# catid/video_stabilizer

Measured on AMD Instinct MI355X. Metric: aligned frames/sec, higher is better.
Workload: dtype u8

## Files before the change

### include/vs_amd.h

```cpp
#ifndef VS_AMD_H
#define VS_AMD_H

#include <stddef.h>
#include <stdint.h>

#ifdef __cplusplus
extern "C" {
#endif

#define VS_OK 0
#define VS_ERR_ARG (-1)
#define VS_ERR_HIP (-2)
#define VS_ERR_UNSUPPORTED (-3)
#define VS_ERR_STATE (-4)
#define VS_ERR_NOMEM (-5)

enum { VS_MEM_HOST = 0, VS_MEM_DEVICE = 1 };
enum { VS_FMT_GRAY8 = 0, VS_FMT_BGR8 = 1, VS_FMT_BGR10 = 2, VS_FMT_BGR12 = 3, VS_FMT_BGR16_FULL = 4 };
int vs_format_bits(int format);
int vs_format_max_value(int format);
enum { VS_WARP_LANCZOS2 = 0, VS_WARP_BILINEAR = 1, VS_WARP_LANCZOS2_FAST = 2, VS_WARP_LANCZOS2_SEP = 3, VS_WARP_BILINEAR_CV = 4 };
enum { VS_BORDER_CLAMP = 0, VS_BORDER_CONSTANT = 1 };
enum {
    VS_SELECT_STL_HOST = 0,
// ... 83 lines not shown
int vs_stream_retire(void* stream);
int vs_bgr_image_warp(const void* src, int w, int h, int src_stride, int channels, int bits,
                      const vs_transform* t, int mode, int border, int max_value,
                      void* dst, int dst_stride, int mem, void* stream);
int vs_bgr_image_warp_batch(const void* src, size_t src_frame_stride, int n_frames,
                            int w, int h, int src_stride, int channels, int bits,
                            const vs_transform* t , int mode, int border, int max_value,
                            void* dst, size_t dst_frame_stride, int dst_stride, int mem, void* stream);
int vs_bgr_image_warp_roi_batch(const void* src, size_t src_frame_stride, int n_frames, int w, int h, int src_stride,
                                int channels, int bits, const vs_transform* t, int mode, int border, int max_value,
                                int roi_x, int roi_y, int roi_w, int roi_h,
                                void* dst, size_t dst_frame_stride, int dst_stride, int mem, void* stream);
int vs_bgr_image_warp_fill_batch(const void* src, size_t src_frame_stride, int n_src, int w, int h, int src_stride,
                                 int channels, int bits, int n_out, int n_cand, const int32_t* cand_frame,
                                 const vs_transform* cand_t, int border, int max_value,
                                 int roi_x, int roi_y, int roi_w, int roi_h,
                                 void* dst, size_t dst_frame_stride, int dst_stride, int mem, void* stream);
typedef struct vs_fill_blend_params { int feather; int match; } vs_fill_blend_params;
int vs_bgr_channel_sums_batch(const void* src, size_t src_frame_stride, int n, int w, int h, int src_stride, int format,
                              uint64_t* sums, int mem, void* stream);
int vs_bgr_image_warp_fill_blend_batch(const void* src, size_t src_frame_stride, int n_src, int w, int h, int src_stride,
                                       int channels, int bits, int n_out, int n_cand, const int32_t* cand_frame,
                                       const vs_transform* cand_t, const uint64_t* sums, const vs_fill_blend_params* params,
                                       int border, int max_value, int roi_x, int roi_y, int roi_w, int roi_h,
                                       void* dst, size_t dst_frame_stride, int dst_stride, int mem, void* stream);
typedef struct vs_deblur_params { float sensitivity; float max_ratio; } vs_deblur_params;
void vs_deblur_params_default(vs_deblur_params* p);
int vs_bgr_sharpness_batch(const void* src, size_t src_frame_stride, int n, int w, int h, int src_stride, int format,
                           uint64_t* sharpness, int mem, void* stream);
int vs_bgr_deblur_batch(const void* src, size_t src_frame_stride, int n_src, int w, int h, int src_stride, int format,
                        const uint64_t* sharpness, int n_out, int n_cand, const int32_t* cand_frame, const vs_transform* cand_t,
                        const vs_deblur_params* params ,
                        void* dst, size_t dst_frame_stride, int dst_stride, int mem, void* stream);
typedef struct vs_denoise_params { int strength; } vs_denoise_params;
void vs_denoise_params_default(vs_denoise_params* p);
int vs_bgr_denoise_batch(const void* src, size_t src_frame_stride, int n_src, int w, int h, int src_stride, int format,
                         int n_out, int n_cand, const int32_t* cand_frame, const vs_transform* cand_t,
                         const vs_denoise_params* params ,
                         void* dst, size_t dst_frame_stride, int dst_stride, int mem, void* stream);
typedef struct vs_deflicker_params { int step; } vs_deflicker_params;
void vs_deflicker_params_default(vs_deflicker_params* p);
int vs_bgr_exposure_stats_batch(const void* src, size_t src_frame_stride, int n_src, int w, int h, int src_stride, int format,
                                int n_out, int n_cand, const int32_t* cand_frame, const vs_transform* cand_t,
                                const vs_deflicker_params* params , uint64_t* stats, int mem, void* stream);
int vs_exposure_gains_batch(const uint64_t* stats, int n_out, int n_cand, int w, int h,
                            const vs_deflicker_params* params , uint32_t* gains, int mem, void* stream);
int vs_bgr_gain_batch(const void* src, size_t src_frame_stride, int n, int w, int h, int src_stride, int format,
                      const uint32_t* gains, void* dst, size_t dst_frame_stride, int dst_stride, int mem, void* stream);
int vs_bgr_image_warp_f32(const void* src, int w, int h, int src_stride, int channels, int bits,
                          const vs_transform* t, int mode, int border,
                          float* dst, int dst_stride, int mem, void* stream);
int vs_bgr_to_gray(const void* src, int w, int h, int src_stride, int bits, int shift_to_8,
                   uint8_t* dst, int dst_stride, int mem, void* stream);

typedef struct vs_flow_params {
    double pyr_scale;
    int    levels;
    int    winsize;
    int    iterations;
    int    poly_n;
    double poly_sigma;
    int    flags;
} vs_flow_params;
void vs_flow_params_default(vs_flow_params* p);
typedef struct vs_flow vs_flow;
vs_flow* vs_flow_create(const vs_flow_params* params , int device);
void     vs_flow_destroy(vs_flow* f);
int vs_flow_compute(vs_flow* f, const uint8_t* prev, const uint8_t* next, int w, int h, int stride, int mem, float* flow,
                    int flow_stride);
int vs_flow_jitter(vs_flow* f, const void* frames, size_t frame_stride, int n, int w, int h, int stride, int format, int mem,
                   float* pair_medians, double* median);

int vs_test_fail_alloc(int k);

int vs_debug_bounds_check(void);
int vs_debug_bounds_selftest(void);

int vs_calib_copy12(const void* src_dev, void* dst_dev, size_t bytes, void* stream);
int vs_shader_clock_probe(void* stream, double* shader_mhz);

typedef struct vs_aligner vs_aligner;
typedef struct vs_align_info {
    int32_t status;
    int32_t fail_reason;
    int32_t fail_level;
    int32_t levels;
    int32_t iterations[16];
    double  condition[16];
    double  phase_dx, phase_dy, phase_response;
    int32_t selected_x[16], selected_y[16];
    vs_transform level_transform[16];
} vs_align_info;

vs_aligner* vs_aligner_create(const vs_aligner_params* params , int device);
void vs_aligner_destroy(vs_aligner* a);
int  vs_aligner_set_select_mode(vs_aligner* a, int select_mode);
int  vs_aligner_get_select_mode(const vs_aligner* a);
enum { VS_BATCH_EXCLUSIVE = 0, VS_BATCH_SHARED = 1 };
int  vs_aligner_set_batch_mode(vs_aligner* a, int batch_mode);
int  vs_aligner_reset(vs_aligner* a);
void* vs_aligner_stream(const vs_aligner* a);
int   vs_aligner_wait_stream(vs_aligner* a, void* producer_stream);
int  vs_aligner_align_next(vs_aligner* a, const void* frame, int w, int h, int stride, int format, int mem,
                           const vs_aligner_params* params, vs_transform* out);
int  vs_aligner_align_batch(vs_aligner* a, const void* frames, size_t frame_stride, int n,
                            int w, int h, int stride, int format, int mem,
// ... 63 lines not shown
```

### video_stabilizer_amd/capi.py

```python
import ctypes as C
import os

import numpy as np

_HERE = os.path.dirname(os.path.abspath(__file__))
LIB_PATH = os.environ.get("VS_AMD_LIB", os.path.join(_HERE, "libvs_amd.so"))

MEM_HOST, MEM_DEVICE = 0, 1
FMT_GRAY8, FMT_BGR8 = 0, 1
FMT_BGR10, FMT_BGR12, FMT_BGR16_FULL = 2, 3, 4
WARP_LANCZOS2, WARP_BILINEAR, WARP_LANCZOS2_FAST, WARP_LANCZOS2_SEP, WARP_BILINEAR_CV = 0, 1, 2, 3, 4
BORDER_CLAMP, BORDER_CONSTANT = 0, 1
SELECT_STL_HOST, SELECT_DEVICE, SELECT_STABLE = 0, 1, 2
BATCH_EXCLUSIVE, BATCH_SHARED = 0, 1
ABI_VERSION = 5


class Transform(C.Structure):
    _fields_ = [("A", C.c_double), ("B", C.c_double), ("TX", C.c_double), ("TY", C.c_double)]

    def tup(self):
        return (self.A, self.B, self.TX, self.TY)

    @staticmethod
# ... 83 lines not shown
    "vs_stabilizer_stream": (_vp, [_vp]),
    "vs_stabilizer_wait_stream": (_i32, [_vp, _vp]),
    "vs_aligner_params_default": (None, [C.POINTER(AlignerParams)]),
    "vs_stabilizer_params_default": (None, [C.POINTER(StabilizerParams)]),
    "vs_transform_inverse": (Transform, [_TP]),
    "vs_transform_compose": (Transform, [_TP, _TP]),
    "vs_transform_warp": (Point, [_TP, Point]),
    "vs_transform_warp_center": (Point, [_TP, Point, _f64, _f64]),
    "vs_transform_max_corner_displacement": (_f64, [_TP, _f64, _f64]),
    "vs_tile_size": (_i32, [_i32, _i32]),
    "vs_ul_params_sparse": (None, [_TP, _i32, _i32, _vp]),
    "vs_ul_params_warp": (None, [_TP, _i32, _i32, _vp]),
    "vs_cv_inverse_matrix": (None, [_TP, _i32, _i32, _vp]),
    "vs_smoother_create": (_vp, [_i32, _i32, _f64]),
    "vs_smoother_destroy": (None, [_vp]),
    "vs_smoother_update": (_i32, [_vp, _TP, _TP]),
    "vs_tvl1_smooth": (None, [_vp, _i32, _f64, _i32, _vp]),
    "vs_calib_copy12": (_i32, [_vp, _vp, _sz, _vp]),
    "vs_pyr_down": (_i32, [_vp, _i32, _i32, _i32, _vp, _i32, _i32, _i32, _i32, _vp]),
    "vs_grad_xy": (_i32, [_vp, _i32, _i32, _i32, _vp, _vp, _i32, _vp]),
    "vs_grad_argmax": (_i32, [_vp, _vp, _i32, _i32, _i32, _vp, _vp, _i32, _vp]),
    "vs_sparse_jac": (_i32, [_vp, _vp, _i32, _i32, _vp, _vp, _i32, _i32, _vp, _vp, _i32, _vp]),
    "vs_keyframe_fused": (_i32, [_vp, _i32, _i32, _i32, _i32, _vp, _vp, _vp, _vp, _i32, _vp]),
    "vs_sparse_warpdiff": (_i32, [_vp, _vp, _i32, _i32, _i32, _vp, _i32, _i32, _f32, _f32, _f32, _f32, _vp, _i32, _vp]),
    "vs_sparse_ica": (_i32, [_vp, _vp, _i32, _i32, _i32, _vp, _i32, _vp, _i32, _vp, _vp, _f32, _f32, _f32, _f32, _vp, _i32, _vp]),
    "vs_select_smallest": (_i32, [_vp, _i32, _i32, _i32, _f32, _vp, _vp, _i32, _vp]),
    "vs_select_smallest_stable": (_i32, [_vp, _i32, _i32, _i32, _f32, _vp, _i32, _vp]),
    "vs_phase_correlate": (_i32, [_vp, _vp, _i32, _i32, _i32, _i32, _vp, _vp, _vp]),
    "vs_optimal_dft_size": (_i32, [_i32]),
    "vs_image_warp": (_i32, [_vp, _i32, _i32, _i32, _f32, _f32, _f32, _f32, _vp, _i32, _i32, _i32, _vp]),
    "vs_bgr_image_warp": (_i32, [_vp, _i32, _i32, _i32, _i32, _i32, _TP, _i32, _i32, _i32, _vp, _i32, _i32, _vp]),
    "vs_bgr_image_warp_batch": (_i32, [_vp, _sz, _i32, _i32, _i32, _i32, _i32, _i32, _TP, _i32, _i32, _i32, _vp, _sz, _i32, _i32, _vp]),
    "vs_bgr_image_warp_roi_batch": (_i32, [_vp, _sz, _i32, _i32, _i32, _i32, _i32, _i32, _TP, _i32, _i32, _i32,
                                           _i32, _i32, _i32, _i32, _vp, _sz, _i32, _i32, _vp]),
    "vs_bgr_image_warp_fill_batch": (_i32, [_vp, _sz, _i32, _i32, _i32, _i32, _i32, _i32, _i32, _i32, C.POINTER(C.c_int32), _TP, _i32, _i32,
                                            _i32, _i32, _i32, _i32, _vp, _sz, _i32, _i32, _vp]),
    "vs_bgr_channel_sums_batch": (_i32, [_vp, _sz, _i32, _i32, _i32, _i32, _i32, _vp, _i32, _vp]),
    "vs_bgr_image_warp_fill_blend_batch": (_i32, [_vp, _sz, _i32, _i32, _i32, _i32, _i32, _i32, _i32, _i32, C.POINTER(C.c_int32), _TP, _vp,
                                                  C.POINTER(FillBlendParams), _i32, _i32, _i32, _i32, _i32, _i32, _vp, _sz, _i32, _i32, _vp]),
    "vs_deblur_params_default": (None, [C.POINTER(DeblurParams)]),
    "vs_bgr_sharpness_batch": (_i32, [_vp, _sz, _i32, _i32, _i32, _i32, _i32, _vp, _i32, _vp]),
    "vs_bgr_deblur_batch": (_i32, [_vp, _sz, _i32, _i32, _i32, _i32, _i32, _vp, _i32, _i32, C.POINTER(C.c_int32), _TP, C.POINTER(DeblurParams),
                                   _vp, _sz, _i32, _i32, _vp]),
    "vs_denoise_params_default": (None, [C.POINTER(DenoiseParams)]),
    "vs_bgr_denoise_batch": (_i32, [_vp, _sz, _i32, _i32, _i32, _i32, _i32, _i32, _i32, C.POINTER(C.c_int32), _TP, C.POINTER(DenoiseParams),
                                    _vp, _sz, _i32, _i32, _vp]),
    "vs_deflicker_params_default": (None, [C.POINTER(DeflickerParams)]),
    "vs_bgr_exposure_stats_batch": (_i32, [_vp, _sz, _i32, _i32, _i32, _i32, _i32, _i32, _i32, C.POINTER(C.c_int32), _TP, C.POINTER(DeflickerParams),
                                           _vp, _i32, _vp]),
    "vs_exposure_gains_batch": (_i32, [_vp, _i32, _i32, _i32, _i32, C.POINTER(DeflickerParams), _vp, _i32, _vp]),
    "vs_bgr_gain_batch": (_i32, [_vp, _sz, _i32, _i32, _i32, _i32, _i32, _vp, _vp, _sz, _i32, _i32, _vp]),
    "vs_bgr_image_warp_f32": (_i32, [_vp, _i32, _i32, _i32, _i32, _i32, _TP, _i32, _i32, _vp, _i32, _i32, _vp]),
    "vs_bgr_to_gray": (_i32, [_vp, _i32, _i32, _i32, _i32, _i32, _vp, _i32, _i32, _vp]),
    "vs_flow_params_default": (None, [C.POINTER(FlowParams)]),
    "vs_flow_create": (_vp, [C.POINTER(FlowParams), _i32]),
    "vs_flow_destroy": (None, [_vp]),
    "vs_flow_compute": (_i32, [_vp, _vp, _vp, _i32, _i32, _i32, _i32, _vp, _i32]),
    "vs_flow_jitter": (_i32, [_vp, _vp, _sz, _i32, _i32, _i32, _i32, _i32, _i32, _vp, C.POINTER(C.c_double)]),
    "vs_aligner_create": (_vp, [C.POINTER(AlignerParams), _i32]),
    "vs_aligner_destroy": (None, [_vp]),
    "vs_aligner_set_select_mode": (_i32, [_vp, _i32]),
    "vs_stabilizer_set_select_mode": (_i32, [_vp, _i32]),
    "vs_aligner_get_select_mode": (_i32, [_vp]),
    "vs_stabilizer_get_select_mode": (_i32, [_vp]),
    "vs_stabilizer_set_border_fill": (_i32, [_vp, _i32]),
    "vs_stabilizer_get_border_fill": (_i32, [_vp]),
    "vs_stabilizer_set_fill_blend": (_i32, [_vp, C.POINTER(FillBlendParams)]),
    "vs_stabilizer_get_fill_blend": (_i32, [_vp, C.POINTER(FillBlendParams)]),
    "vs_stabilizer_set_deblur": (_i32, [_vp, _i32, C.POINTER(DeblurParams)]),
    "vs_stabilizer_get_deblur": (_i32, [_vp]),
    "vs_stabilizer_set_denoise": (_i32, [_vp, _i32, C.POINTER(DenoiseParams)]),
    "vs_stabilizer_get_denoise": (_i32, [_vp]),
    "vs_stabilizer_set_deflicker": (_i32, [_vp, _i32, C.POINTER(DeflickerParams)]),
    "vs_stabilizer_get_deflicker": (_i32, [_vp]),
    "vs_aligner_set_batch_mode": (_i32, [_vp, _i32]),
    "vs_aligner_reset": (_i32, [_vp]),
    "vs_aligner_align_next": (_i32, [_vp, _vp, _i32, _i32, _i32, _i32, _i32, C.POINTER(AlignerParams), _TP]),
    "vs_aligner_align_batch": (_i32, [_vp, _vp, _sz, _i32, _i32, _i32, _i32, _i32, _i32, C.POINTER(AlignerParams), _TP, C.POINTER(C.c_int32)]),
    "vs_aligner_align_clips": (_i32, [_vp, _vp, _sz, _i32, _i32, _i32, _i32, _i32, _i32, _i32, C.POINTER(AlignerParams), _TP, C.POINTER(C.c_int32)]),
    "vs_aligner_enable_timing": (_i32, [_vp, _i32]),
    "vs_aligner_get_timings": (_i32, [_vp, C.POINTER(StageTimings)]),
    "vs_aligner_get_info": (_i32, [_vp, _i32, C.POINTER(AlignInfo)]),
    "vs_aligner_level_dims": (_i32, [_vp, _i32, _IP, _IP, _IP, _IP, _IP]),
    "vs_aligner_read_level_image": (_i32, [_vp, _i32, _i32, _vp]),
    "vs_aligner_read_level_argmax": (_i32, [_vp, _i32, _i32, _i32, _vp]),
    "vs_aligner_read_level_jacobian": (_i32, [_vp, _i32, _i32, _i32, _vp]),
    "vs_stabilizer_create": (_vp, [C.POINTER(StabilizerParams), _i32]),
    "vs_stabilizer_destroy": (None, [_vp]),
    "vs_stabilizer_process": (_i32, [_vp, _vp, _i32, _i32, _i32, _i32, _i32, _vp, _IP, _IP]),
    "vs_stabilizer_process_batch": (_i32, [_vp, _vp, _sz, _i32, _i32, _i32, _i32, _i32, _i32, _vp, _sz, C.POINTER(C.c_int32), _IP, _IP]),
    "vs_stabilizer_process_clips": (_i32, [_vp, _vp, _sz, _i32, _i32, _i32, _i32, _i32, _i32, _i32, _vp, _sz, C.POINTER(C.c_int32), _IP, _IP]),
    "vs_stabilizer_reset": (_i32, [_vp]),
    "vs_stabilizer_state": (None, [_vp, _TP, _TP, _IP]),
}

_lib = None


def lib():
    global _lib
    if _lib is not None:
        return _lib
    if not os.path.exists(LIB_PATH):
        raise VsError("libvs_amd.so is missing (%s): run `python -c 'import __graft_entry__ as g; g.build()'`" % LIB_PATH)
    L = C.CDLL(LIB_PATH)
    partial = os.environ.get("VS_AMD_LIB_PARTIAL") == "1"
# ... 496 lines not shown
    out = np.full((n_out, 4), 0xA5A5A5A5, np.uint32)
    _check(lib().vs_exposure_gains_batch(_p(st), n_out, n_cand, w, h, C.byref(params) if params is not None else None, _p(out), MEM_HOST, None))
    return out


def exposure_gains_batch_device(stats_ptr, n_out, n_cand, w, h, gains_ptr, params=None, stream=None):
    _check(lib().vs_exposure_gains_batch(_p(stats_ptr), n_out, n_cand, w, h, C.byref(params) if params is not None else None, _p(gains_ptr), MEM_DEVICE,
                                         C.c_void_p(stream) if stream else None))


def bgr_gain_batch(src, gains, fmt=None, src_stride=None, dst_stride=None, guard=None):
    src = np.ascontiguousarray(src)
    n, h, w, c = src.shape
    fmt = _fmt_of(src.dtype, 3) if fmt is None else fmt
    ss = w * c if src_stride is None else src_stride
    ds = w * c if dst_stride is None else dst_stride
    buf = _pitched(src, ss)
    g = _c(gains, np.uint32)
    out = np.full((n, h, ds), 0 if guard is None else guard, src.dtype)
    _check(lib().vs_bgr_gain_batch(_p(buf), h * ss, n, w, h, ss, fmt, _p(g), _p(out), h * ds, ds, MEM_HOST, None))
    res = np.ascontiguousarray(out[:, :, :w * c]).reshape(n, h, w, c)
    return (res, out) if guard is not None else res


def bgr_gain_batch_device(src_ptr, src_fs, n, w, h, src_stride, fmt, gains_ptr, dst_ptr, dst_fs, dst_stride, stream=None):
    _check(lib().vs_bgr_gain_batch(_p(src_ptr), src_fs, n, w, h, src_stride, fmt, _p(gains_ptr), _p(dst_ptr), dst_fs, dst_stride, MEM_DEVICE,
                                   C.c_void_p(stream) if stream else None))


def sharpness_batch_device(src_ptr, n, w, h, fmt, sharp_ptr, stream=None):
    _check(lib().vs_bgr_sharpness_batch(_p(src_ptr), h * w * 3, n, w, h, w * 3, fmt, _p(sharp_ptr), MEM_DEVICE, C.c_void_p(stream) if stream else None))


def bgr_image_warp_batch_device(src_ptr, n, w, h, c, bits, ts, dst_ptr, mode=WARP_LANCZOS2, border=BORDER_CLAMP,
                                max_value=None, stream=None):
    if max_value is None:
        max_value = 255 if bits == 8 else 65535
    arr = ts if isinstance(ts, C.Array) else (Transform * n)(*ts)
    _check(lib().vs_bgr_image_warp_batch(_p(src_ptr), h * w * c, n, w, h, w * c, c, bits, arr, mode, border, max_value,
                                         _p(dst_ptr), h * w * c, w * c, MEM_DEVICE, stream))


def bgr_to_gray(src, shift_to_8=None):
    src = np.ascontiguousarray(src)
    h, w, _ = src.shape
    bits = 8 if src.dtype == np.uint8 else 16
    if shift_to_8 is None:
        shift_to_8 = 0 if bits == 8 else 2
    out = np.empty((h, w), np.uint8)
    _check(lib().vs_bgr_to_gray(_p(src), w, h, w * 3, bits, shift_to_8, _p(out), w, MEM_HOST, None))
    return out


def _fmt_of(frame_dtype, ndim_tail):
    if ndim_tail == 2:
        return FMT_GRAY8
    return FMT_BGR8 if frame_dtype == np.uint8 else FMT_BGR10


def flow_params(**kw):
    p = FlowParams()
    lib().vs_flow_params_default(C.byref(p))
    for k, v in kw.items():
        if not hasattr(p, k):
            raise TypeError("FlowParams has no field %r" % k)
        setattr(p, k, v)
    return p


class Flow:

    def __init__(self, params=None, device=0):
        self.params = params if params is not None else flow_params()
        self.h = lib().vs_flow_create(C.byref(self.params), device)
        if not self.h:
            raise VsError("vs_flow_create failed: %s" % lib().vs_last_error().decode())

    def compute(self, prev, next_):
        a = np.asarray(prev)
        b = np.asarray(next_)
        if a.dtype != np.uint8 or b.dtype != np.uint8 or a.ndim != 2 or a.shape != b.shape:
            raise ValueError("dense_flow takes two u8 gray images of the same shape")
        if a.strides[1] != 1 or b.strides[1] != 1 or a.strides[0] != b.strides[0]:
            a, b = np.ascontiguousarray(a), np.ascontiguousarray(b)
        h, w = a.shape
        out = np.empty((h, w, 2), np.float32)
        _check(lib().vs_flow_compute(self.h, _p(a), _p(b), w, h, a.strides[0], MEM_HOST, _p(out), 2 * w))
        return out

    def jitter(self, frames, fmt=None):
        frames = np.ascontiguousarray(frames)
        n = frames.shape[0]
        fmt = _fmt_of(frames.dtype, frames.ndim - 1) if fmt is None else fmt
        hh, ww = frames.shape[1:3]
        ch = 1 if fmt == FMT_GRAY8 else 3
        pm = np.zeros(max(n - 1, 0), np.float32)
        med = C.c_double(0.0)
        _check(lib().vs_flow_jitter(self.h, _p(frames), hh * ww * ch, n, ww, hh, ww * ch, fmt, MEM_HOST, _p(pm), C.byref(med)))
        return med.value, pm

    def jitter_device(self, ptr, n, w, h, fmt, stride=None, frame_stride=None):
        ch = 1 if fmt == FMT_GRAY8 else 3
        stride = stride or w * ch
        frame_stride = frame_stride or h * stride
        pm = np.zeros(max(n - 1, 0), np.float32)
        med = C.c_double(0.0)
# ... 265 lines not shown
```

### video_stabilizer_amd/csrc/vs_capi.hip

```cpp
#include "vs_internal.hpp"
#include "vs_kernels.hpp"
#include "vs_phase.hpp"

#include <algorithm>
#include <atomic>
#include <new>
#include <cstdio>
#include <cstdlib>
#include <cstring>
#include <deque>
#include <mutex>
#include <vector>

namespace vsi {

bool device_ready() {
    int n = 0;
    hipError_t e = hipGetDeviceCount(&n);
    if (e != hipSuccess || n <= 0) {
        set_error(VS_ERR_HIP, "no usable HIP device (%s): libvs_amd has no CPU fallback",
                  e == hipSuccess ? "device count 0" : hipGetErrorString(e));
        return false;
    }
    return true;
// ... 929 lines not shown
int vs_bgr_image_warp_fill_batch(const void* src, size_t src_fs, int n_src, int w, int h, int src_stride, int channels, int bits, int n_out, int n_cand,
                                 const int32_t* cand_frame, const vs_transform* cand_t, int border, int max_value, int roi_x, int roi_y, int roi_w,
                                 int roi_h, void* dst, size_t dst_fs, int dst_stride, int mem, void* stream) try {
    return fill_batch_impl(src, src_fs, n_src, w, h, src_stride, channels, bits, n_out, n_cand, cand_frame, cand_t, border, max_value, roi_x, roi_y, roi_w, roi_h,
                           dst, dst_fs, dst_stride, mem, stream, nullptr, nullptr);
} VS_CATCH_ALL

int vs_bgr_image_warp_fill_blend_batch(const void* src, size_t src_fs, int n_src, int w, int h, int src_stride, int channels, int bits, int n_out, int n_cand,
                                       const int32_t* cand_frame, const vs_transform* cand_t, const uint64_t* sums, const vs_fill_blend_params* params,
                                       int border, int max_value, int roi_x, int roi_y, int roi_w, int roi_h, void* dst, size_t dst_fs, int dst_stride,
                                       int mem, void* stream) try {
    VS_ARG(params);
    return fill_batch_impl(src, src_fs, n_src, w, h, src_stride, channels, bits, n_out, n_cand, cand_frame, cand_t, border, max_value, roi_x, roi_y, roi_w, roi_h,
                           dst, dst_fs, dst_stride, mem, stream, sums, params);
} VS_CATCH_ALL

int vs_bgr_channel_sums_batch(const void* src, size_t src_fs, int n, int w, int h, int src_stride, int format, uint64_t* sums, int mem, void* stream) try {
    VS_DIMS(w, h);
    int bits = 0;
    VS_TRY(bgr_format_ok(format, &bits));
    VS_ARG(src && sums && n >= 1 && w >= 1 && h >= 1 && src_stride >= w * 3);
    if (w > 32767 || h > 32767) return set_error(VS_ERR_UNSUPPORTED, "channel sums: frames up to 32767 x 32767, as the border fill");
    VS_ARG(n == 1 || src_fs >= img_span(w, h, src_stride, 3));
    if (!vsi::device_ready()) return VS_ERR_HIP;
    hipStream_t s = (hipStream_t)stream;
    const size_t esz = bits > 8 ? 2 : 1;
    Staged a, o;
    VS_TRY(a.in(src, ((size_t)(n - 1) * src_fs + img_span(w, h, src_stride, 3)) * esz, mem, s));
    VS_TRY(o.out(sums, (size_t)n * 3 * sizeof(uint64_t), mem));
    VS_HIP(vsk::bgr_channel_sums(a.dev, w, h, src_stride, (int)esz * 8, o.as<unsigned long long>(), n, src_fs, s));
    return vsi::finish_outputs(mem, s, {&o});
} VS_CATCH_ALL

int vs_bgr_image_warp_f32(const void* src, int w, int h, int src_stride, int channels, int bits, const vs_transform* t,
                          int mode, int border, float* dst, int dst_stride, int mem, void* stream) try {
    return bgr_warp_common(src, 0, 1, w, h, src_stride, channels, bits, t, mode, border, 0, dst, 0, dst_stride, true, mem,
                           (hipStream_t)stream);
} VS_CATCH_ALL

int vs_bgr_to_gray(const void* src, int w, int h, int src_stride, int bits, int shift_to_8, uint8_t* dst, int dst_stride,
                   int mem, void* stream) try {
    VS_DIMS(w, h);
    VS_ARG(src && dst && w > 0 && h > 0 && src_stride >= 3 * w && dst_stride >= w && (bits == 8 || bits == 16));
    VS_ARG(shift_to_8 >= 0 && shift_to_8 <= 8);
    if (!vsi::device_ready()) return VS_ERR_HIP;
    hipStream_t s = (hipStream_t)stream;
    Staged a, o;
    VS_TRY(a.in(src, img_span(w, h, src_stride, 3) * (bits / 8), mem, s));
    VS_TRY(o.out_image(dst, (size_t)w, (size_t)h, (size_t)dst_stride, 1, 0, mem));
    VS_HIP(vsk::bgr_to_gray(a.dev, w, h, src_stride, bits, shift_to_8, o.as<uint8_t>(), dst_stride, 1, 0, 0, s));
    return vsi::finish_outputs(mem, s, {&o});
} VS_CATCH_ALL


int vs_bgr_sharpness_batch(const void* src, size_t src_fs, int n, int w, int h, int src_stride, int format, uint64_t* sharpness, int mem,
                           void* stream) try {
    VS_DIMS(w, h);
    int bits = 0;
    VS_TRY(bgr_format_ok(format, &bits));
    VS_ARG(src && sharpness && n >= 1 && src_stride >= w * 3);
    VS_ARG(n == 1 || src_fs >= img_span(w, h, src_stride, 3));
    if (!vsi::device_ready()) return VS_ERR_HIP;
    hipStream_t s = (hipStream_t)stream;
    const size_t esz = bits > 8 ? 2 : 1;
    Staged a, o;
    VS_TRY(a.in(src, ((size_t)(n - 1) * src_fs + img_span(w, h, src_stride, 3)) * esz, mem, s));
    VS_TRY(o.out(sharpness, (size_t)n * sizeof(uint64_t), mem));
    VS_HIP(vsk::bgr_sharpness(a.dev, w, h, src_stride, (int)esz * 8, bits - 8, o.as<unsigned long long>(), n, src_fs, s));
    return vsi::finish_outputs(mem, s, {&o});
} VS_CATCH_ALL

static int deblur_params_ok(const vs_deblur_params* params, vs_deblur_params* p) {
    if (params) *p = *params; else vs_deblur_params_default(p);
    VS_ARG(vsi::deblur_params_finite(p->sensitivity, p->max_ratio));
    return VS_OK;
}

int vsi::bgr_deblur_ptrs(int n_out, int w, int h, int src_stride, int format, int n_cand, const void* const* cand_src, const uint64_t* const* cand_sharp,
                         const vs_transform* cand_t, const vs_deblur_params* params, void* dst, size_t dst_fs, int dst_stride, hipStream_t s) {
    VS_DIMS(w, h);
    int bits = 0;
    VS_TRY(bgr_format_ok(format, &bits));
    VS_ARG(cand_src && cand_sharp && cand_t && dst && n_out >= 1 && n_cand >= 1 && n_cand <= 16 && src_stride >= w * 3 && dst_stride >= w * 3);
    VS_ARG(n_out == 1 || dst_fs >= img_span(w, h, dst_stride, 3));
    vs_deblur_params p;
    VS_TRY(deblur_params_ok(params, &p));
    ParamRing* ring = param_ring();
    if (!ring) return set_error(VS_ERR_HIP, "no parameter ring for this device");
    const size_t esz = bits > 8 ? 2 : 1;
    const char* const fn = __func__;
    std::vector<vsk::DeblurCand> dc;
    return cand_groups(ring, 0, n_out, std::max(1, (int)(ParamRing::kSlots / 2 / 5) / n_cand), n_cand, cand_src, cand_t, w, h, true, true, s, dc,
        [&](vsk::DeblurCand& e, int o) -> int {
            const size_t base = (size_t)o * n_cand;
            VS_ARG_AS(cand_src[base] && cand_sharp[base], fn);
            e.src = cand_src[base];
            e.sharp = (const unsigned long long*)cand_sharp[base];
            return VS_OK;
        },
        [&](vsk::DeblurCand& e, size_t k) { return (e.sharp = (const unsigned long long*)cand_sharp[k]) != nullptr; },
        [&](vsk::DeblurCand* cdev, float* rdev, int f0, int nf) -> int {
            VS_HIP(vsk::bgr_deblur(cdev, rdev, n_cand, w, h, src_stride, (int)esz * 8, bits - 8, vs_format_max_value(format), p.sensitivity, p.max_ratio,
                                   (char*)dst + (size_t)f0 * dst_fs * esz, dst_stride, nf, dst_fs, targets_aligned(cand_src, f0, nf, n_cand), s));
            return VS_OK;
        });
}
// ... 190 lines not shown
```

### video_stabilizer_amd/csrc/vs_kernels.hip

```cpp
#include "vs_kernels.hpp"
#include <cstdlib>
#include <algorithm>

#include <utility>
#include "vs_device.hpp"

using namespace vsd;

namespace {
constexpr int PD_TW = 64, PD_TH = 16;
constexpr int PD_IW = 2 * PD_TW + 8;
constexpr int PD_IH = 2 * PD_TH + 3;
constexpr int PD_IWP = PD_IW;
}

__device__ __forceinline__ void pyr_passes(const uint8_t (*tile)[PD_IWP], uint32_t (*hsum)[PD_TW / 2], int x0, int y0,
                                           uint8_t* __restrict__ out, int ow, int oh, int out_stride) {
    for (int i = threadIdx.x; i < PD_IH * (PD_TW / 2); i += 256) {
        const int r = i >> 5, p = i & 31;
        const uint32_t* row = (const uint32_t*)&tile[r][0];
        const uint32_t d0 = row[p], d1 = row[p + 1], d2 = row[p + 2];
        uint32_t h0 = __builtin_amdgcn_udot4(__builtin_amdgcn_alignbyte(d1, d0, 2), 0x04060401u, 0u, false);
        h0 = __builtin_amdgcn_udot4(d1, 0x00010000u, h0, false);
        uint32_t h1 = __builtin_amdgcn_udot4(d1, 0x04060401u, 0u, false);
// ... 265 lines not shown
        if (interior) {
            const uint32_t o_own = (__umul24((uint32_t)(iy0 + r_own), (uint32_t)src_stride) + (uint32_t)(gx_own * 3)) * (uint32_t)sizeof(T);
            const uint32_t o_step = 8u * (uint32_t)src_stride * (uint32_t)sizeof(T);
#pragma unroll
            for (int it = 0; it < 4; it++) load_group_at(q[it], o_own + (uint32_t)it * o_step);
            load_group_at(q[4], (__umul24((uint32_t)(iy0 + r_h), (uint32_t)src_stride) + (uint32_t)(gx_h * 3)) * (uint32_t)sizeof(T));
            const uint32_t g_own = __umul24((uint32_t)(iy0 + r_own), (uint32_t)w) + (uint32_t)gx_own, g_step = 8u * (uint32_t)w;
            const int t_own = r_own * (PD_IWP / 4) + c_own;
#pragma unroll
            for (int it = 0; it < 4; it++) {
                const uint32_t v = gray_word(q[it]);
                tile_w[t_own + 8 * it * (PD_IWP / 4)] = v;
                *(uint32_t*)(g0 + (g_own + (uint32_t)it * g_step)) = v;
            }
            if (has_halo) tile_w[r_h * (PD_IWP / 4) + c_h] = gray_word(q[4]);
        } else {
#pragma unroll
        for (int it = 0; it < 4; it++) load_group(q[it], min(iy0 + r_own + 8 * it, h - 1), gxc_own);
        load_group(q[4], clampi(iy0 + r_h, 0, h - 1), gxc_h);
        const bool own_border = gx_own != gxc_own, own_dword = g0_aligned && gx_own + 3 < w;
        const uint32_t own_sel = border_sel(gx_own, gxc_own);
#pragma unroll
        for (int it = 0; it < 4; it++) {
            uint32_t v = gray_word(q[it]);
            if (own_border) v = __builtin_amdgcn_perm(0u, v, own_sel);
            const int r = r_own + 8 * it, oy = iy0 + r;
            tile_w[r * (PD_IWP / 4) + c_own] = v;
            if (oy < h && gx_own < w) {
                uint8_t* dst = g0 + (__umul24((uint32_t)oy, (uint32_t)w) + (uint32_t)gx_own);
                if (own_dword) *(uint32_t*)dst = v;
                else for (int k = 0; k < 4 && gx_own + k < w; k++) dst[k] = (uint8_t)(v >> (8 * k));
            }
        }
        if (has_halo) {
            uint32_t v = gray_word(q[4]);
            if (gx_h != gxc_h) v = __builtin_amdgcn_perm(0u, v, border_sel(gx_h, gxc_h));
            tile_w[r_h * (PD_IWP / 4) + c_h] = v;
        }
        }
    } else {
        for (int i = threadIdx.x; i < N_ITEMS; i += 256) {
            const int r = i / (PD_IW / 4), c4 = (i - r * (PD_IW / 4)) * 4;
            const int gy = clampi(iy0 + r, 0, h - 1), gx = ix0 + c4;
            const T* row = src + (size_t)gy * src_stride;
            uint32_t v = 0;
#pragma unroll
            for (int k = 0; k < 4; k++) v |= gray_of(row + (size_t)clampi(gx + k, 0, w - 1) * 3, shift_to_8) << (8 * k);
            stage(r, c4, gx, v);
        }
    }
    __syncthreads();
    pyr_passes(tile, hsum, x0, y0, g1, ow, oh, ow);
    }
    }
}

__global__ __launch_bounds__(256) void vs_k_grad_xy(const uint8_t* __restrict__ in, int w, int h, int stride,
                                                    float* __restrict__ gx, float* __restrict__ gy) {
    const int x = blockIdx.x * 256 + threadIdx.x, y = blockIdx.y;
    if (x >= w) return;
    const uint8_t* row = in + (size_t)y * stride;
    float l = (float)row[max(x - 1, 0)], r = (float)row[min(x + 1, w - 1)];
    float u = (float)in[(size_t)max(y - 1, 0) * stride + x], d = (float)in[(size_t)min(y + 1, h - 1) * stride + x];
    gx[(size_t)y * w + x] = 0.5f * (r - l);
    gy[(size_t)y * w + x] = 0.5f * (d - u);
}

__global__ __launch_bounds__(256) void vs_k_grad_argmax(const float* __restrict__ gx, const float* __restrict__ gy,
                                                        int w, int h, int ts, int tx, int ty,
                                                        uint16_t* __restrict__ lmx, uint16_t* __restrict__ lmy) {
    const int tile = blockIdx.x * 4 + (threadIdx.x >> 6), lane = threadIdx.x & 63;
    if (tile >= tx * ty) return;
    const int tyi = tile / tx, txi = tile % tx;
    const int bx = txi * ts, by = tyi * ts, n = ts * ts;
    unsigned long long kx = 0, ky = 0;
    for (int i = lane; i < n; i += 64) {
        int ry = i / ts, rx = i % ts;
        size_t o = (size_t)(by + ry) * w + (bx + rx);
        unsigned long long inv = 0xffffffffu - (unsigned)i;
        unsigned long long a = ((unsigned long long)__float_as_uint(fabsf(gx[o])) << 32) | inv;
        unsigned long long b = ((unsigned long long)__float_as_uint(fabsf(gy[o])) << 32) | inv;
        kx = a > kx ? a : kx;
        ky = b > ky ? b : ky;
    }
    kx = wave_max_u64(kx);
    ky = wave_max_u64(ky);
    if (lane == 0) {
        const size_t nt = (size_t)tx * ty;
        int ix = (int)(0xffffffffu - (unsigned)(kx & 0xffffffffu)), iy = (int)(0xffffffffu - (unsigned)(ky & 0xffffffffu));
        lmx[tile] = (uint16_t)(bx + ix % ts);
        lmx[nt + tile] = (uint16_t)(by + ix / ts);
        lmy[tile] = (uint16_t)(bx + iy % ts);
        lmy[nt + tile] = (uint16_t)(by + iy / ts);
    }
}

__global__ __launch_bounds__(256) void vs_k_sparse_jac(const float* __restrict__ gx, const float* __restrict__ gy,
                                                       int w, int h, const uint16_t* __restrict__ lmx,
                                                       const uint16_t* __restrict__ lmy, int nt,
                                                       float* __restrict__ jx, float* __restrict__ jy) {
    const int i = blockIdx.x * 256 + threadIdx.x;
    if (i >= nt) return;
    const float cx = (float)w * 0.5f, cy = (float)h * 0.5f, scale = 1.f / (float)w;
    int ix0 = min((int)lmx[i], w - 1), iy0 = min((int)lmx[nt + i], h - 1);
    int ix1 = min((int)lmy[i], w - 1), iy1 = min((int)lmy[nt + i], h - 1);
    float u0 = (float)ix0 - cx, v0 = (float)iy0 - cy, u1 = (float)ix1 - cx, v1 = (float)iy1 - cy;
// ... 435 lines not shown
                              (float)v11 * ((float)(a1 * b1) * k);
            r = (int)rintf(sum);
        }
        dst[(size_t)y * dst_stride + (size_t)x * channels + c] = (T)min(max(r, 0), max_value);
    }
}

__global__ __launch_bounds__(256) void vs_k_calib_copy12(const uint32_t* __restrict__ src, uint32_t* __restrict__ dst,
                                                         size_t n_groups) {
    typedef uint32_t u32x3 __attribute__((ext_vector_type(3)));
    for (size_t i = (size_t)blockIdx.x * 256 + threadIdx.x; i < n_groups; i += (size_t)gridDim.x * 256)
        *(u32x3*)(dst + 3 * i) = *(const u32x3*)(src + 3 * i);
}

namespace vsk {

static inline int cdiv(int a, int b) { return (a + b - 1) / b; }

hipError_t calib_copy12(const void* src, void* dst, size_t bytes, hipStream_t s) {
    hipLaunchKernelGGL(vs_k_calib_copy12, dim3(4096), dim3(256), 0, s, (const uint32_t*)src, (uint32_t*)dst, bytes / 12);
    return hipGetLastError();
}

hipError_t pyr_down(const uint8_t* in, int w, int h, int in_stride, uint8_t* out, int ow, int oh, int out_stride,
                    int n_frames, size_t in_fs, size_t out_fs, hipStream_t s) {
    if (ow <= 0 || oh <= 0 || n_frames <= 0) return hipSuccess;
    const int strips_x = cdiv(ow, 2 * PR_LIVE);
    const int bands = cdiv(oh, n_frames <= 4 ? 4 : PR_OUT);
    const dim3 grid(cdiv(strips_x * bands, 4), n_frames);
#define VS_PD(ROWS, NARROW)                                                                                             \
    hipLaunchKernelGGL((vs_k_pyr_down_rows<ROWS, NARROW>), grid, dim3(256), 0, s, in, w, h, in_stride, out, ow, oh, out_stride, in_fs, \
                       out_fs, strips_x, bands)
    if (n_frames <= 4) { if (w < 4) VS_PD(4, true); else VS_PD(4, false); }
    else { if (w < 4) VS_PD(PR_OUT, true); else VS_PD(PR_OUT, false); }
#undef VS_PD
    return hipGetLastError();
}

hipError_t bgr_to_gray(const void* src, int w, int h, int src_stride, int bits, int shift_to_8, uint8_t* dst,
                       int dst_stride, int n_frames, size_t src_fs, size_t dst_fs, hipStream_t s) {
    dim3 grid(cdiv(w, 1024), h, n_frames);
    if (bits == 8)
        hipLaunchKernelGGL(vs_k_bgr_to_gray<uint8_t>, grid, dim3(256), 0, s, (const uint8_t*)src, w, h, src_stride,
                           shift_to_8, dst, dst_stride, src_fs, dst_fs);
    else
        hipLaunchKernelGGL(vs_k_bgr_to_gray<uint16_t>, grid, dim3(256), 0, s, (const uint16_t*)src, w, h, src_stride,
                           shift_to_8, dst, dst_stride, src_fs, dst_fs);
    return hipGetLastError();
}

hipError_t ingest_pyr(const void* src, int w, int h, int src_stride, int bits, int shift_to_8, uint8_t* g0, uint8_t* g1,
                      int n_frames, size_t src_fs, size_t pyr_fs, hipStream_t s) {
    const int ow = w / 2, oh = h / 2;
    const int tiles_x = cdiv(w, 2 * PD_TW), tiles_y = cdiv(h, 2 * PD_TH);
    const long long tpf = (long long)tiles_x * tiles_y;
    if (tpf > 0x3fffffLL || tiles_x > 1024) return hipErrorNotSupported;
    const int chunk = (int)((tpf + 7) / 8);
    const uint32_t magic = (uint32_t)(0x100000000ULL / (uint32_t)tiles_x) + 1u;
    const size_t esz = bits == 8 ? 1 : 2;
    for (int f0 = 0; f0 < n_frames; f0 += 65535) {
        const int nf = std::min(65535, n_frames - f0);
        const dim3 grid((unsigned)(chunk * 8), (unsigned)nf);
        const uint8_t* sp = (const uint8_t*)src + (size_t)f0 * src_fs * esz;
        if (bits == 8)
            hipLaunchKernelGGL(vs_k_ingest_pyr<uint8_t>, grid, dim3(256), 0, s, (const uint8_t*)sp, w, h, src_stride, shift_to_8,
                               g0 + (size_t)f0 * pyr_fs, g1 + (size_t)f0 * pyr_fs, ow, oh, src_fs, pyr_fs, tiles_x, magic, (int)tpf, chunk);
        else
            hipLaunchKernelGGL(vs_k_ingest_pyr<uint16_t>, grid, dim3(256), 0, s, (const uint16_t*)sp, w, h, src_stride, shift_to_8,
                               g0 + (size_t)f0 * pyr_fs, g1 + (size_t)f0 * pyr_fs, ow, oh, src_fs, pyr_fs, tiles_x, magic, (int)tpf, chunk);
    }
    return hipGetLastError();
}

hipError_t grad_xy(const uint8_t* in, int w, int h, int stride, float* gx, float* gy, hipStream_t s) {
    hipLaunchKernelGGL(vs_k_grad_xy, dim3(cdiv(w, 256), h), dim3(256), 0, s, in, w, h, stride, gx, gy);
    return hipGetLastError();
}

hipError_t grad_argmax(const float* gx, const float* gy, int w, int h, int ts, uint16_t* lmx, uint16_t* lmy,
                       hipStream_t s) {
    int tx = w / ts, ty = h / ts;
    if (tx * ty == 0) return hipSuccess;
    hipLaunchKernelGGL(vs_k_grad_argmax, dim3(cdiv(tx * ty, 4)), dim3(256), 0, s, gx, gy, w, h, ts, tx, ty, lmx, lmy);
    return hipGetLastError();
}

hipError_t sparse_jac(const float* gx, const float* gy, int w, int h, const uint16_t* lmx, const uint16_t* lmy,
                      int nt, float* jx, float* jy, hipStream_t s) {
    if (nt == 0) return hipSuccess;
    hipLaunchKernelGGL(vs_k_sparse_jac, dim3(cdiv(nt, 256)), dim3(256), 0, s, gx, gy, w, h, lmx, lmy, nt, jx, jy);
    return hipGetLastError();
}

hipError_t keyframe(const uint8_t* img, int w, int h, int stride, int ts, uint16_t* lmx, uint16_t* lmy, float* jx,
                    float* jy, int n_frames, size_t img_fs, size_t lm_fs, size_t jac_fs, hipStream_t s, bool aos) {
    int tx = w / ts, ty = h / ts;
    if (tx * ty == 0) return hipSuccess;
#define VS_ROWS(TS)                                                                                                     \
    case TS: {                                                                                                          \
        constexpr int tpw = keyframe_rows_tiles_per_wave(TS);                                                           \
        const int strips_x = cdiv(tx, tpw);                                                                             \
        hipLaunchKernelGGL(vs_k_keyframe_rows<TS>, dim3(cdiv(strips_x * ty, 4), n_frames), dim3(256), 0, s, img, w, h,  \
                           stride, tx, ty, lmx, lmy, jx, jy, img_fs, lm_fs, jac_fs, strips_x, aos);                     \
        break;                                                                                                          \
    }
    switch (ts) {
// ... 96 lines not shown
```

Baseline: 89770.

## Add wave-per-strip row-streaming ingest kernel for gray conversion and pyramid level

```diff
diff --git a/include/vs_amd.h b/include/vs_amd.h
--- a/include/vs_amd.h
+++ b/include/vs_amd.h
@@ -159,6 +159,8 @@
                           float* dst, int dst_stride, int mem, void* stream);
 int vs_bgr_to_gray(const void* src, int w, int h, int src_stride, int bits, int shift_to_8,
                    uint8_t* dst, int dst_stride, int mem, void* stream);
+int vs_ingest_pyr(const void* src, size_t src_frame_stride, int n, int w, int h, int src_stride, int format,
+                  uint8_t* pyr, size_t level1_offset, size_t pyr_frame_stride, int mem, void* stream);
 
 typedef struct vs_flow_params {
     double pyr_scale;
diff --git a/video_stabilizer_amd/capi.py b/video_stabilizer_amd/capi.py
--- a/video_stabilizer_amd/capi.py
+++ b/video_stabilizer_amd/capi.py
@@ -159,6 +159,7 @@
     "vs_bgr_gain_batch": (_i32, [_vp, _sz, _i32, _i32, _i32, _i32, _i32, _vp, _vp, _sz, _i32, _i32, _vp]),
     "vs_bgr_image_warp_f32": (_i32, [_vp, _i32, _i32, _i32, _i32, _i32, _TP, _i32, _i32, _vp, _i32, _i32, _vp]),
     "vs_bgr_to_gray": (_i32, [_vp, _i32, _i32, _i32, _i32, _i32, _vp, _i32, _i32, _vp]),
+    "vs_ingest_pyr": (_i32, [_vp, _sz, _i32, _i32, _i32, _i32, _i32, _vp, _sz, _sz, _i32, _vp]),
     "vs_flow_params_default": (None, [C.POINTER(FlowParams)]),
     "vs_flow_create": (_vp, [C.POINTER(FlowParams), _i32]),
     "vs_flow_destroy": (None, [_vp]),
@@ -761,6 +762,28 @@
     return out
 
 
+def ingest_pyr(frames, fmt=None, src_stride=None, src_frame_stride=None, level1_offset=None, pyr_frame_stride=None, fill=0xA5):
+    if isinstance(frames, tuple):
+        flat, (n, h, w) = frames
+        flat = np.ascontiguousarray(flat)
+        dtype = flat.dtype
+    else:
+        flat = np.ascontiguousarray(frames)
+        n, h, w = flat.shape[:3]
+        dtype = flat.dtype
+    fmt = (FMT_BGR8 if dtype == np.uint8 else FMT_BGR10) if fmt is None else fmt
+    src_stride = src_stride or 3 * w
+    src_frame_stride = src_frame_stride or h * src_stride
+    ow, oh = w // 2, h // 2
+    level1_offset = level1_offset or w * h
+    pyr_frame_stride = pyr_frame_stride or level1_offset + ow * oh
+    pyr = np.full((n, pyr_frame_stride), fill, np.uint8)
+    _check(lib().vs_ingest_pyr(_p(flat), src_frame_stride, n, w, h, src_stride, fmt, _p(pyr), level1_offset, pyr_frame_stride, MEM_HOST, None))
+    l0 = [pyr[i, :w * h].reshape(h, w) for i in range(n)]
+    l1 = [pyr[i, level1_offset:level1_offset + ow * oh].reshape(oh, ow) for i in range(n)]
+    return pyr, l0, l1
+
+
 def _fmt_of(frame_dtype, ndim_tail):
     if ndim_tail == 2:
         return FMT_GRAY8
diff --git a/video_stabilizer_amd/csrc/vs_capi.hip b/video_stabilizer_amd/csrc/vs_capi.hip
--- a/video_stabilizer_amd/csrc/vs_capi.hip
+++ b/video_stabilizer_amd/csrc/vs_capi.hip
@@ -1005,6 +1005,29 @@
     return vsi::finish_outputs(mem, s, {&o});
 } VS_CATCH_ALL
 
+int vs_ingest_pyr(const void* src, size_t src_fs, int n, int w, int h, int src_stride, int format, uint8_t* pyr, size_t level1_offset,
+                  size_t pyr_fs, int mem, void* stream) try {
+    VS_DIMS(w, h);
+    int bits = 0;
+    VS_TRY(bgr_format_ok(format, &bits));
+    VS_ARG(src && pyr && n >= 1 && n <= 65535 && src_stride >= w * 3);
+    VS_ARG(n == 1 || src_fs >= img_span(w, h, src_stride, 3));
+    VS_ARG(level1_offset >= (size_t)w * h && level1_offset < ((size_t)1 << 32) && pyr_fs >= level1_offset + (size_t)(w / 2) * (h / 2));
+    if (!vsi::device_ready()) return VS_ERR_HIP;
+    hipStream_t s = (hipStream_t)stream;
+    const size_t esz = bits > 8 ? 2 : 1;
+    Staged a, o;
+    VS_TRY(a.in(src, ((size_t)(n - 1) * src_fs + img_span(w, h, src_stride, 3)) * esz, mem, s));
+    VS_TRY(o.out(pyr, (size_t)n * pyr_fs, mem));
+    if (o.staged) {
+        memcpy(o.blk->pin, pyr, o.bytes);
+        VS_HIP(hipMemcpyAsync(o.dev, o.blk->pin, o.bytes, hipMemcpyHostToDevice, s));
+    }
+    VS_HIP(vsk::ingest_pyr(a.dev, w, h, src_stride, (int)esz * 8, bits - 8, o.as<uint8_t>(), o.as<uint8_t>() + level1_offset, n, src_fs,
+                           pyr_fs, s));
+    return vsi::finish_outputs(mem, s, {&o});
+} VS_CATCH_ALL
+
 
 int vs_bgr_sharpness_batch(const void* src, size_t src_fs, int n, int w, int h, int src_stride, int format, uint64_t* sharpness, int mem,
                            void* stream) try {
diff --git a/video_stabilizer_amd/csrc/vs_kernels.hip b/video_stabilizer_amd/csrc/vs_kernels.hip
--- a/video_stabilizer_amd/csrc/vs_kernels.hip
+++ b/video_stabilizer_amd/csrc/vs_kernels.hip
@@ -341,6 +341,131 @@
     __syncthreads();
     pyr_passes(tile, hsum, x0, y0, g1, ow, oh, ow);
     }
+    }
+}
+
+namespace {
+constexpr int IR_LIVE = 62;
+constexpr int IR_OUT = 16;
+constexpr bool kIngestRowsDefault = true;
+}
+
+template <typename T>
+__device__ __forceinline__ uint32_t ingest_gray_word(const uint32_t* q, int shift_to_8) {
+    if (sizeof(T) == 1) {
+        constexpr uint32_t kH = (3735u >> 7) | ((19235u >> 7) << 8) | ((9798u >> 7) << 16);
+        constexpr uint32_t kL = (2u * (3735u & 127u)) | ((2u * (19235u & 127u)) << 8) | ((2u * (9798u & 127u)) << 16);
+        const uint32_t px[4] = {q[0], __builtin_amdgcn_alignbyte(q[1], q[0], 3), __builtin_amdgcn_alignbyte(q[2], q[1], 2), q[2] >> 8};
+        uint32_t t[4];
+#pragma unroll
+        for (int k = 0; k < 4; k++)
+            t[k] = (__builtin_amdgcn_udot4(px[k], kH, 0u, false) << 8) + __builtin_amdgcn_udot4(px[k], kL, 32768u, false);
+        const uint32_t t01 = __builtin_amdgcn_perm(t[1], t[0], 0x0c0c0602u), t23 = __builtin_amdgcn_perm(t[3], t[2], 0x0c0c0602u);
+        return __builtin_amdgcn_perm(t23, t01, 0x05040100u);
+    }
+    const uint32_t bg[4] = {q[0], __builtin_amdgcn_alignbyte(q[2], q[1], 2), q[3], __builtin_amdgcn_alignbyte(q[5], q[4], 2)};
+    const uint32_t rr[4] = {q[1] & 0xffffu, q[2] >> 16, q[4] & 0xffffu, q[5] >> 16};
+    constexpr uint32_t kWBG = 3735u | (19235u << 16);
+    uint32_t v = 0;
+#pragma unroll
+    for (int k = 0; k < 4; k++) {
+        const uint32_t t = __builtin_amdgcn_udot2(__builtin_bit_cast(us2, bg[k]), __builtin_bit_cast(us2, kWBG), 16384u, false);
+        uint32_t g = ((t + rr[k] * 9798u) >> 15) >> shift_to_8;
+        g = g > 255u ? 255u : g;
+        v |= g << (8 * k);
+    }
+    return v;
+}
+
+template <typename T>
+__global__ __launch_bounds__(256) void vs_k_ingest_rows(const T* __restrict__ src_all, int w, int h, int src_stride, int shift_to_8,
+                                                        uint8_t* __restrict__ g0_all, uint8_t* __restrict__ g1_all, int ow, int oh,
+                                                        size_t src_frame_stride, size_t pyr_frame_stride, int strips_x,
+                                                        uint32_t strips_x_magic, int jobs_per_frame, int chunk) {
+    const int wave = __builtin_amdgcn_readfirstlane((int)(threadIdx.x >> 6)), lane = threadIdx.x & 63;
+    const int job = ((int)(blockIdx.x & 7) * chunk + (int)(blockIdx.x >> 3)) * 4 + wave;
+    if (job >= jobs_per_frame) return;
+    const int band = strips_x == 1 ? job : (int)__umulhi((uint32_t)job, strips_x_magic);
+    const int strip = job - band * strips_x;
+    const uint8_t* __restrict__ src = (const uint8_t*)(src_all + (size_t)blockIdx.y * src_frame_stride);
+    uint8_t* __restrict__ g0 = g0_all + (size_t)blockIdx.y * pyr_frame_stride;
+    uint8_t* __restrict__ g1 = g1_all + (size_t)blockIdx.y * pyr_frame_stride;
+    constexpr int QW = sizeof(T) == 1 ? 3 : 6;
+    constexpr int D = sizeof(T) == 1 ? 4 : 2;
+
+    const int x_first = strip * (IR_LIVE * 4);
+    const int n_live = min(IR_LIVE, (w - x_first + 3) >> 2);
+    const int x0 = x_first + (lane - 1) * 4, ox = x0 >> 1, oy0 = band * IR_OUT;
+    const bool live = lane >= 1 && lane <= n_live;
+    auto word_off = [&](int l) { return l <= 0 ? max(x_first - 4, 0) : min(x_first + (min(l, n_live + 1) - 1) * 4, w - 4); };
+    const int off_o = word_off(lane), off_l = word_off(lane - 1), off_r = word_off(lane + 1);
+    auto sel = [&](int c, int hi, int lo) -> unsigned {
+        c = min(max(c, 0), w - 1);
+        const unsigned d = (unsigned)(c - lo);
+        return d < 4u ? d : 4u + ((unsigned)(c - hi) & 3u);
+    };
+    const unsigned sel_l = sel(x0 - 2, off_o, off_l) | (sel(x0 - 1, off_o, off_l) << 8) | (sel(x0, off_o, off_l) << 16) |
+                           (sel(x0 + 1, off_o, off_l) << 24);
+    const unsigned sel_m = sel(x0, off_o, off_o) | (sel(x0 + 1, off_o, off_o) << 8) | (sel(x0 + 2, off_o, off_o) << 16) |
+                           (sel(x0 + 3, off_o, off_o) << 24);
+    const unsigned sel_e = 0x0c000c00u | sel(x0 + 2, off_r, off_o) | (sel(x0 + 4, off_r, off_o) << 16);
+    const uint32_t lane_src = (uint32_t)(off_o * 3) * (uint32_t)sizeof(T);
+    const bool live1 = live && ox < ow, two = ox + 1 < ow;
+
+    const int y_own = 2 * oy0, y_end = min(y_own + 2 * IR_OUT, h);
+    const int rows_out = min(IR_OUT, oh - oy0);
+    const int y_last = y_own + 2 * rows_out;
+    auto load_row = [&](uint32_t (&q)[QW], int y) {
+        const int yc = min(max(__builtin_amdgcn_readfirstlane(min(y, y_last)), 0), h - 1);
+        const uint32_t* gp = (const uint32_t*)(src + ((uint32_t)(yc * src_stride) * (uint32_t)sizeof(T) + lane_src));
+        if (sizeof(T) == 1) {
+            typedef uint32_t u32x3 __attribute__((ext_vector_type(3)));
+            const u32x3 t = *(const u32x3*)gp;
+            q[0] = t.x; q[1] = t.y; q[2] = t.z;
+        } else {
+            typedef uint32_t u32x2 __attribute__((ext_vector_type(2)));
+            typedef uint32_t u32x4 __attribute__((ext_vector_type(4)));
+            const u32x4 ta = *(const u32x4*)gp;
+            const u32x2 tb = *(const u32x2*)(gp + 4);
+            q[0] = ta.x; q[1] = ta.y; q[2] = ta.z; q[3] = ta.w; q[QW - 2] = tb.x; q[QW - 1] = tb.y;
+        }
+    };
+    auto hrow = [&](const uint32_t (&q)[QW], int y) -> us2 {
+        const uint32_t own = ingest_gray_word<T>(q, shift_to_8);
+        if (y >= y_own && y < y_end) {
+            if (live) __builtin_memcpy(g0 + ((uint32_t)(y * w) + (uint32_t)off_o), &own, 4);
+        }
+        const uint32_t left = (uint32_t)dpp_mov0<0x138>((int)own);
+        const uint32_t right = (uint32_t)dpp_mov0<0x130>((int)own);
+        const uint32_t l4 = __builtin_amdgcn_perm(own, left, sel_l);
+        const uint32_t m4 = __builtin_amdgcn_perm(own, own, sel_m);
+        const uint32_t e2 = __builtin_amdgcn_perm(right, own, sel_e);
+        const uint32_t lo = __builtin_amdgcn_udot4(l4, 0x04060401u, e2, false);
+        return __builtin_bit_cast(us2, (__builtin_amdgcn_udot4(m4, 0x04060401u, 0u, false) << 16) + lo);
+    };
+    uint32_t head[3][QW], ring[D][QW];
+#pragma unroll
+    for (int j = 0; j < 3; j++) load_row(head[j], y_own - 2 + j);
+#pragma unroll
+    for (int j = 0; j < D; j++) load_row(ring[j], y_own + 1 + j);
+    us2 h0 = hrow(head[0], y_own - 2), h1 = hrow(head[1], y_own - 1), h2 = hrow(head[2], y_own);
+#pragma unroll 1
+    for (int r0 = 0; r0 < rows_out; r0 += D / 2) {
+#pragma unroll
+        for (int j = 0; j < D / 2; j++) {
+            const int r = r0 + j, ya = y_own + 1 + 2 * r;
+            const us2 h3 = hrow(ring[2 * j], ya), h4 = hrow(ring[2 * j + 1], ya + 1);
+            load_row(ring[2 * j], ya + D);
+            load_row(ring[2 * j + 1], ya + 1 + D);
+            const us2 v = (h0 + h4) + (h1 + h3) * (unsigned short)4 + h2 * (unsigned short)6;
+            const uint32_t packed = __builtin_amdgcn_perm(0u, __builtin_bit_cast(uint32_t, v), 0x0c0c0301u);
+            if (r < rows_out && live1) {
+                uint8_t* dst = g1 + ((uint32_t)((oy0 + r) * ow) + (uint32_t)ox);
+                if (two) { const uint16_t t = (uint16_t)packed; __builtin_memcpy(dst, &t, 2); }
+                else dst[0] = (uint8_t)packed;
+            }
+            h0 = h2; h1 = h3; h2 = h4;
+        }
     }
 }
 
@@ -882,6 +1007,31 @@
 hipError_t ingest_pyr(const void* src, int w, int h, int src_stride, int bits, int shift_to_8, uint8_t* g0, uint8_t* g1,
                       int n_frames, size_t src_fs, size_t pyr_fs, hipStream_t s) {
     const int ow = w / 2, oh = h / 2;
+    const size_t esz_in = bits == 8 ? 1 : 2;
+    static const bool rows_env = []() { const char* e = getenv("VS_INGEST_ROWS"); return e ? atoi(e) != 0 : kIngestRowsDefault; }();
+    const bool rows_ok = ((((uintptr_t)src) | ((uintptr_t)src_stride * esz_in) | (n_frames > 1 ? (uintptr_t)(src_fs * esz_in) : 0)) & 3u) == 0 &&
+                         w >= 4 && h >= 1 && w < (1 << 24) && h < (1 << 24) && src_stride < (1 << 24) &&
+                         (unsigned long long)h * (unsigned long long)src_stride * esz_in < (1ull << 31);
+    if (rows_env && rows_ok) {
+        const int strips_x = cdiv(w, 4 * IR_LIVE), bands = cdiv(h, 2 * IR_OUT);
+        const long long jobs = (long long)strips_x * bands;
+        if (jobs * strips_x < 0x100000000LL) {
+            const int chunk = (int)((cdiv((int)jobs, 4) + 7) / 8);
+            const uint32_t magic = (uint32_t)(0x100000000ULL / (uint32_t)strips_x) + 1u;
+            for (int f0 = 0; f0 < n_frames; f0 += 65535) {
+                const int nf = std::min(65535, n_frames - f0);
+                const dim3 grid((unsigned)(chunk * 8), (unsigned)nf);
+                const uint8_t* sp = (const uint8_t*)src + (size_t)f0 * src_fs * esz_in;
+                if (bits == 8)
+                    hipLaunchKernelGGL(vs_k_ingest_rows<uint8_t>, grid, dim3(256), 0, s, (const uint8_t*)sp, w, h, src_stride, shift_to_8,
+                                       g0 + (size_t)f0 * pyr_fs, g1 + (size_t)f0 * pyr_fs, ow, oh, src_fs, pyr_fs, strips_x, magic, (int)jobs, chunk);
+                else
+                    hipLaunchKernelGGL(vs_k_ingest_rows<uint16_t>, grid, dim3(256), 0, s, (const uint16_t*)sp, w, h, src_stride, shift_to_8,
+                                       g0 + (size_t)f0 * pyr_fs, g1 + (size_t)f0 * pyr_fs, ow, oh, src_fs, pyr_fs, strips_x, magic, (int)jobs, chunk);
+            }
+            return hipGetLastError();
+        }
+    }
     const int tiles_x = cdiv(w, 2 * PD_TW), tiles_y = cdiv(h, 2 * PD_TH);
     const long long tpf = (long long)tiles_x * tiles_y;
     if (tpf > 0x3fffffLL || tiles_x > 1024) return hipErrorNotSupported;
```

Result: slower. 88240 (-1.7%).
